# alexrenz/AdaPM

Measured on AMD Instinct MI355X. Metric: pull_push_ops_per_s, higher is better.
Workload: dtype fp32; 1 GPU; model=kge_complex_dim512, entities=10000000, relations=1000, dim=512, neg_samples=16, global_batch=16384, triples=90000000, parallelism=ps-async-dp1, fused_step=True, warmup_extra_steps=400

## Files before the change

### adapm_amd/csrc/core.cpp

```cpp
#include <torch/extension.h>
#include <ATen/Parallel.h>

#include <algorithm>
#include <atomic>
#include <condition_variable>
#include <cstring>
#include <limits>
#include <deque>
#include <map>
#include <queue>
#include <tuple>
#include <memory>
#include <mutex>
#include <random>
#include <thread>
#include <chrono>
#include <unordered_map>
#include <unordered_set>
#include <cstdio>
#include <vector>

#include "common.h"
#include "kernels.h"
#include "ops.h"
// ... 2385 lines not shown
  std::string failed_reason() {
    std::lock_guard<std::mutex> g(tickets_mu_);
    return failed_reason_;
  }

  void sync_finish(int ch, bool globally_idle = false) {
    if (globally_idle) {
      std::lock_guard<std::mutex> g(channels_[ch].mu);
      if (!channels_[ch].responses.empty()) globally_idle = false;
      for (const auto& r : channels_[ch].out_queue) {
        bool data = (r.payload.defined() && r.payload.numel() > 0) ||
                    r.code == M_PUSH_REQ || r.code == M_SET_REQ || r.code == M_PUSH_REQ_BULK;
        if (data) {
          globally_idle = false;
          break;
        }
      }
    }
    {
      std::lock_guard<std::mutex> g(rounds_mu_);
      ChannelState& C = channels_[ch];
      C.rounds++;
      if (globally_idle) {
        if (++C.idle_streak >= 2) C.idle2_events++;
      } else {
        C.idle_streak = 0;
      }
    }
    rounds_cv_.notify_all();
  }

  py::dict debug_pending() {
    py::dict d;
    {
      std::lock_guard<std::mutex> g(tickets_mu_);
      d["tickets"] = tickets_.size();
    }
    py::list outq, respq, rounds;
    for (auto& C : channels_) {
      std::lock_guard<std::mutex> g(C.mu);
      outq.append(C.out_queue.size());
      respq.append(C.responses.size());
      rounds.append(C.rounds.load());
    }
    d["out_queues"] = outq;
    d["responses"] = respq;
    d["rounds"] = rounds;
    return d;
  }


  bool fused_plain_ok(void* st) {
    if (clocks_.size() != 1 || fused_multi_stream_) return false;
    if (!fused_marks_.defined()) {
      if (getenv("ADAPM_FUSED_ATOMIC")) {
        fused_multi_stream_ = true;
        return false;
      }
      fused_marks_ = torch::zeros({rowmark_words(num_keys_)},
                                  torch::TensorOptions().dtype(torch::kInt32).device(dev_));
      if (getenv("ADAPM_FUSED_STATS"))
        fused_shared_stat_ =
            torch::zeros({1}, torch::TensorOptions().dtype(torch::kInt64).device(dev_));
      fused_marks_stream_ = st;
      return true;
    }
    if (st == fused_marks_stream_) return true;
#ifdef ADAPM_WITH_HIP
    hipStreamSynchronize((hipStream_t)fused_marks_stream_);
#endif
    fused_multi_stream_ = true;
    return false;
  }

  void check_fused_identity(const char* name, int64_t D) {
    TORCH_CHECK(world_ == 1, name, " requires a single rank (all keys local)");
    TORCH_CHECK(uniform_len_ == 2 * D, name, ": store rows must be [emb|accum] = 2D");
    TORCH_CHECK(layout_identity_.load(), name, " requires the identity layout");
    TORCH_CHECK(dev_.is_cuda(), name, " is the GPU fast path");
  }

  void count_fused_ops(int64_t keys) {
    stat_pull_keys_ += keys;
    stat_pull_local_ += keys;
    stat_push_keys_ += keys;
    stat_push_local_ += keys;
    stat_pulls_ += 1;
    stat_pushes_ += 1;
  }

  struct StagedKeys {
    torch::Tensor dev;
    std::vector<const int64_t*> ptr;
  };
  StagedKeys stage_keys(const char* name, std::initializer_list<const torch::Tensor*> parts) {
    int64_t total = 0;
    for (auto* t : parts) {
      check_keys(*t);
      total += t->numel();
    }
    auto blob = torch::empty(
        {total}, torch::TensorOptions().dtype(torch::kInt64).pinned_memory(true));
    int64_t* dst = blob.data_ptr<int64_t>();
    const uint64_t lim = (uint64_t)num_keys_;
    uint64_t bad = 0;
    for (auto* t : parts) {
      const int64_t* kp = t->data_ptr<int64_t>();
      const int64_t n = t->numel();
      for (int64_t i = 0; i < n; ++i) {
        int64_t k = kp[i];
        dst[i] = k;
        bad |= ((uint64_t)k >= lim);
      }
      dst += n;
    }
    if (bad)
      for (auto* t : parts) check_key_range(*t);
    StagedKeys sk;
    sk.dev = torch::empty({total}, torch::TensorOptions().dtype(torch::kInt64).device(dev_));
#ifdef ADAPM_WITH_HIP
    auto stream = c10::hip::getCurrentHIPStreamMasqueradingAsCUDA(dev_.index());
    TORCH_CHECK(copy_keys_gpu(sk.dev.data_ptr<int64_t>(), blob.data_ptr<int64_t>(), total,
                              (void*)stream.stream()),
                name, ": the pinned key staging buffer is not visible to the device");
    at::getHostAllocator(at::kCUDA)->record_event(
        blob.data_ptr(), blob.storage().data_ptr().get_context(), stream.unwrap());
#else
    TORCH_CHECK(false, name, ": built without HIP");
#endif
    const int64_t* dp = sk.dev.data_ptr<int64_t>();
    for (auto* t : parts) {
      sk.ptr.push_back(dp);
      dp += t->numel();
    }
    return sk;
  }

  std::tuple<torch::Tensor, torch::Tensor> kge_step_fused_impl(
      const torch::Tensor& keys_s, const torch::Tensor& keys_r, const torch::Tensor& keys_o,
      const torch::Tensor* keys_neg, UniformStream* us, int64_t N, int64_t D, double lr,
      double eps) {
    check_fused_identity("kge_step_fused", D);
    check_step_lanes("kge_step_fused", "D/2", D / 2);
    int64_t B = keys_s.numel();
    TORCH_CHECK(keys_r.numel() == B && keys_o.numel() == B);
    StagedKeys sk;
    torch::Tensor drawn;
    const int64_t* kn;
    if (us) {
      TORCH_CHECK(us->lo() >= 0 && us->hi() <= num_keys_, "kge_step_fused_sampled: stream range [",
                  us->lo(), ", ", us->hi(), ") exceeds the store's ", num_keys_, " keys");
      TORCH_CHECK(us->device() == dev_,
                  "kge_step_fused_sampled: stream is not on the store's device");
      TORCH_CHECK(N >= 0 && B * N > 0, "kge_step_fused_sampled: nothing to draw");
      sk = stage_keys("kge_step_fused", {&keys_s, &keys_r, &keys_o});
      drawn = us->draw(B * N);
      kn = drawn.data_ptr<int64_t>();
    } else {
      TORCH_CHECK(keys_neg->numel() == B * N);
      sk = stage_keys("kge_step_fused", {&keys_s, &keys_r, &keys_o, keys_neg});
      kn = sk.ptr[3];
    }
    const int64_t *ks = sk.ptr[0], *kr = sk.ptr[1], *ko = sk.ptr[2];

    auto loss = torch::empty({B}, torch::TensorOptions().dtype(torch::kFloat32).device(dev_));
    void* st = current_stream(dev_);
    {
      InflightGuard g(this);
      std::unique_lock<std::mutex> mg(fused_mu_);
      if (fused_plain_ok(st)) {
        RowMarkKeys mk{{ks, kr, ko, kn}, {B, B, B, B * N}, 4};
        auto* marks = reinterpret_cast<uint32_t*>(fused_marks_.data_ptr<int32_t>());
        rowmark_set_gpu(marks, mk, st);
        kge_complex_step_fused_gpu(
            slab_.data, mk.keys[0], mk.keys[1], mk.keys[2], mk.keys[3], loss.data_ptr<float>(),
            (int)B, (int)N, (int)D, Slab::padded(uniform_len_), world_, (float)lr, (float)eps,
            st, marks,
            fused_shared_stat_.defined()
                ? reinterpret_cast<unsigned long long*>(fused_shared_stat_.data_ptr<int64_t>())
                : nullptr);
        rowmark_clear_gpu(marks, mk, st);
        stat_fused_plain_ += 1;
      } else {
        mg.unlock();
        kge_complex_step_fused_gpu(slab_.data, ks, kr, ko, kn, loss.data_ptr<float>(), (int)B,
                                   (int)N, (int)D, Slab::padded(uniform_len_), world_, (float)lr,
                                   (float)eps, st);
        stat_fused_atomic_ += 1;
      }
    }
    count_fused_ops(3 * B + B * N);
    return {loss, drawn};
  }

  torch::Tensor kge_step_fused(torch::Tensor keys_s, torch::Tensor keys_r, torch::Tensor keys_o,
                               torch::Tensor keys_neg, int64_t N, int64_t D, double lr,
                               double eps) {
    return std::get<0>(
        kge_step_fused_impl(keys_s, keys_r, keys_o, &keys_neg, nullptr, N, D, lr, eps));
  }

  std::tuple<torch::Tensor, torch::Tensor> kge_step_fused_sampled(
      torch::Tensor keys_s, torch::Tensor keys_r, torch::Tensor keys_o, UniformStream& us,
      int64_t N, int64_t D, double lr, double eps) {
    return kge_step_fused_impl(keys_s, keys_r, keys_o, nullptr, &us, N, D, lr, eps);
  }

  struct FusedResolve {
    std::vector<std::vector<int64_t>> offs;
    std::vector<int64_t> missed;
    int64_t b_hit = 0;
    std::vector<const int64_t*> ptr;
    std::vector<torch::Tensor> dev;
  };

  FusedResolve resolve_fused(const std::vector<std::pair<const int64_t*, int>>& arrs,
                             int64_t B) {
    FusedResolve out;
    const int na = (int)arrs.size();
    constexpr int64_t G = 1024;
    int64_t nchunks = (B + G - 1) / G;
    struct Part {
      std::vector<std::vector<int64_t>> offs;
      std::vector<int64_t> missed;
    };
    std::vector<Part> parts(nchunks);
    pass_pool_.run(nchunks, [&](int64_t c0, int64_t c1) {
      for (int64_t c = c0; c < c1; ++c) {
        Part& P = parts[c];
        P.offs.resize(na);
        int64_t e = std::min(B, (c + 1) * G);
        std::vector<int64_t> tmp;
        for (int64_t b = c * G; b < e; ++b) {
          tmp.clear();
          bool ok = true;
          for (int a = 0; a < na && ok; ++a) {
            const int64_t* kp = arrs[a].first;
            int cnt = arrs[a].second;
            for (int i = 0; i < cnt; ++i) {
              Key k = kp[b * cnt + i];
// ... 563 lines not shown
  std::vector<ChannelState> channels_;
  std::unique_ptr<std::atomic<uint16_t>[]> intent_cnt_;
  std::vector<std::atomic<Clock>> clocks_;
  Clock intent_ahead_ = 1LL << 40;

  std::atomic<bool> layout_identity_{true};

  std::atomic<int> inflight_{0};
  int max_hops_ = getenv("ADAPM_MAX_HOPS") ? atoi(getenv("ADAPM_MAX_HOPS")) : 64;
  PassPool pass_pool_;
  std::atomic<int> migrating_{0};
  double sync_threshold_ = 0.0;
  std::unique_ptr<std::atomic<uint32_t>[]> heat_;
  std::mutex spill_mu_;
  std::mutex rebalance_mu_;
  std::vector<Key> spill_touched_;
  int64_t rebalance_calls_ = 0;
  std::atomic<int64_t> stat_spill_moves_{0};
  std::atomic<int64_t> next_ts_{1};
 public:
  std::atomic<int64_t> t_pass_{0}, t_todev_{0}, t_launch_{0}, t_calls_{0}, t_misc_{0};
  std::atomic<int64_t> t_sy_intents_{0}, t_sy_replicas_{0}, t_sy_build_{0}, t_sy_proc_{0},
      t_sy_apply_{0}, n_sy_deltas_{0}, n_sy_proc_recs_{0}, n_sy_apply_recs_{0};
  bool cpp_timing_ = getenv("ADAPM_CPP_TIMING") != nullptr;
 private:
  std::mutex tickets_mu_;
  std::condition_variable tickets_cv_;
  std::unordered_map<int64_t, std::unique_ptr<Ticket>> tickets_;
  std::unordered_map<int64_t, std::string> failed_tickets_;
  std::string failed_reason_;
  std::atomic<bool> failed_flag_{false};
  std::mutex rounds_mu_;
  std::condition_variable rounds_cv_;

  bool locality_stats_ = false;
  std::vector<std::atomic<uint32_t>> key_accesses_, key_local_;
  std::mutex trace_mu_;
  std::unordered_set<Key> traced_keys_;
  bool trace_all_ = false;
  struct TraceEv { double t; Key k; const char* ev; };
  std::vector<TraceEv> trace_;
  std::chrono::steady_clock::time_point t0_ = std::chrono::steady_clock::now();

  std::atomic<int64_t> hop_hist_[9] = {};
  std::atomic<int64_t> stat_replica_records_{0}, stat_replica_payloads_{0};
  std::atomic<int64_t> stat_pulls_{0}, stat_pushes_{0}, stat_pull_keys_{0}, stat_push_keys_{0},
      stat_pull_local_{0}, stat_push_local_{0}, stat_pull_replica_{0}, stat_push_replica_{0},
      stat_remote_pulls_served_{0}, stat_remote_pushes_served_{0}, stat_relocations_{0},
      stat_relocated_in_{0}, stat_replications_{0}, stat_drops_{0}, stat_forwards_{0},
      stat_dropped_records_{0}, stat_delta_overhops_{0}, stat_bytes_sent_{0},
      stat_bytes_recv_{0}, stat_sampling_checks_{0};

  std::mutex fused_mu_;
  torch::Tensor fused_marks_;
  torch::Tensor fused_shared_stat_;
  void* fused_marks_stream_ = nullptr;
  bool fused_multi_stream_ = false;
  std::atomic<int64_t> stat_fused_plain_{0}, stat_fused_atomic_{0};
};


static float* fp(torch::Tensor& t) { return t.data_ptr<float>(); }
static const float* cfp(const torch::Tensor& t) { return t.data_ptr<float>(); }

static void check_f32(const torch::Tensor& t, const char* name) {
  TORCH_CHECK(t.is_contiguous() && t.scalar_type() == torch::kFloat32, name,
              " must be contiguous float32");
}

void kge_complex_step(torch::Tensor s, torch::Tensor r, torch::Tensor o, torch::Tensor neg,
                      torch::Tensor ds, torch::Tensor dr, torch::Tensor do_, torch::Tensor dneg,
                      torch::Tensor loss, int64_t N, int64_t D, double lr, double eps) {
  for (auto* t : {&s, &r, &o, &neg, &ds, &dr, &do_, &dneg, &loss}) check_f32(*t, "kge tensor");
  int B = (int)loss.numel();
  if (s.is_cuda()) {
    TORCH_CHECK(hip_available(), "kge_complex_step: CUDA tensor but no HIP device");
    check_step_lanes("kge_complex_step", "D/2", D / 2);
    kge_complex_step_gpu(cfp(s), cfp(r), cfp(o), cfp(neg), fp(ds), fp(dr), fp(do_), fp(dneg),
                         fp(loss), B, (int)N, (int)D, (float)lr, (float)eps,
                         current_stream(s.device()));
  } else {
    kge_complex_step_cpu(cfp(s), cfp(r), cfp(o), cfp(neg), fp(ds), fp(dr), fp(do_), fp(dneg),
                         fp(loss), B, (int)N, (int)D, (float)lr, (float)eps);
  }
}

void rescal_step(torch::Tensor s, torch::Tensor r, torch::Tensor o, torch::Tensor neg,
                 torch::Tensor ds, torch::Tensor drl, torch::Tensor do_, torch::Tensor dneg,
                 torch::Tensor loss, int64_t N, int64_t D, double lr, double eps) {
  for (auto* t : {&s, &r, &o, &neg, &ds, &drl, &do_, &dneg, &loss}) check_f32(*t, "rescal");
  int B = (int)loss.numel();
  TORCH_CHECK(D <= 196, "rescal_step: dim must be <= 196 (R tile staged in LDS)");
  if (s.is_cuda()) {
    TORCH_CHECK(hip_available(), "rescal_step: CUDA tensor but no HIP device");
    rescal_step_gpu(cfp(s), cfp(r), cfp(o), cfp(neg), fp(ds), fp(drl), fp(do_), fp(dneg),
                    fp(loss), B, (int)N, (int)D, (float)lr, (float)eps,
                    current_stream(s.device()));
  } else {
    rescal_step_cpu(cfp(s), cfp(r), cfp(o), cfp(neg), fp(ds), fp(drl), fp(do_), fp(dneg),
                    fp(loss), B, (int)N, (int)D, (float)lr, (float)eps);
  }
}

void kge_complex_score(torch::Tensor s, torch::Tensor r, torch::Tensor cand,
                       torch::Tensor scores, int64_t D) {
  for (auto* t : {&s, &r, &cand, &scores}) check_f32(*t, "kge tensor");
  int B = (int)scores.size(0), E = (int)scores.size(1);
  if (s.is_cuda()) {
    TORCH_CHECK(hip_available(), "kge_complex_score: CUDA tensor but no HIP device");
// ... 214 lines not shown
  auto up = [&](const torch::Tensor& t) { return gpu ? t.to(dev.device()) : t; };
  torch::Tensor s_d = up(src_off), d_d = up(dst_off), l_d = up(lens), a_d;
  if (has_aux) a_d = up(*aux_off);
  OpsBatch b{s_d.data_ptr<int64_t>(), d_d.data_ptr<int64_t>(), l_d.data_ptr<int32_t>(), (int)n};
  const int64_t* a = has_aux ? a_d.data_ptr<int64_t>() : nullptr;
  float* bp = has_buf ? buf->data_ptr<float>() : nullptr;
  void* st = current_stream(dev.device());
  switch (kind) {
    case GATHER: gpu ? ops_gather_gpu(sb, b, bp, st) : ops_gather_cpu(sb, b, bp); break;
    case SCATTER: gpu ? ops_scatter_gpu(sb, b, bp, set, st) : ops_scatter_cpu(sb, b, bp, set); break;
    case RMW: ops_scatter_rmw_gpu(sb, b, bp, st); break;
    case EXTRACT: gpu ? ops_extract_gpu(sb, b, a, bp, st) : ops_extract_cpu(sb, b, a, bp); break;
    case REFRESH: gpu ? ops_refresh_gpu(sb, b, a, bp, st) : ops_refresh_cpu(sb, b, a, bp); break;
    case ZERO: gpu ? ops_zero_gpu(sb, b, st) : ops_zero_cpu(sb, b); break;
    case SQNORM: gpu ? ops_delta_sqnorm_gpu(sb, b, a, bp, st) : ops_delta_sqnorm_cpu(sb, b, a, bp); break;
  }
}

void slab_keys_op(const std::string& op, torch::Tensor dev, torch::Tensor keys, int64_t len,
                  int64_t plen, int64_t world, int64_t rank, torch::Tensor buf, bool set) {
  const bool gather = op == "gather_keys";
  TORCH_CHECK(gather || op == "scatter_keys", "slab_keys_op: unknown op '", op, "'");
  TORCH_CHECK(!(gather && set), "slab_keys_op: set applies to scatter_keys only");
  const bool gpu = dev.is_cuda();
  TORCH_CHECK(!gpu || hip_available(), "slab_keys_op: CUDA tensor but no HIP device");
  check_slab_tensor(dev, torch::kFloat32, "dev slab");
  check_slab_tensor(buf, torch::kFloat32, "buf");
  TORCH_CHECK(buf.device() == dev.device(), "slab_keys_op: buf and dev on different devices");
  const int64_t n = keys.numel();
  check_host_batch_tensor(keys, torch::kInt64, n, "keys");
  TORCH_CHECK(n <= std::numeric_limits<int>::max(), "slab_keys_op: batch too large");
  TORCH_CHECK(len >= 1 && plen >= len && plen <= std::numeric_limits<int32_t>::max(),
              "slab_keys_op: need 1 <= len <= plen");
  TORCH_CHECK((len & 3) != 0 || (plen & 3) == 0, "slab_keys_op: len % 4 == 0 needs plen % 4 == 0");
  TORCH_CHECK(world >= 1 && rank >= 0 && rank < world, "slab_keys_op: bad world / rank");
  TORCH_CHECK(n * len <= buf.numel(), "slab_keys_op: buf holds fewer than n rows");
  const int64_t* kp = keys.data_ptr<int64_t>();
  const int64_t rows = dev.numel() / plen;
  for (int64_t i = 0; i < n; ++i) {
    TORCH_CHECK(kp[i] >= 0, "slab_keys_op: keys[", i, "] is negative");
    TORCH_CHECK(kp[i] % world != rank || kp[i] / world < rows, "slab_keys_op: keys[", i, "] = ",
                kp[i], " lies past the slab's ", rows, " slots");
  }
  torch::Tensor k_d = gpu ? keys.to(dev.device()) : keys;
  SlabBases sb{dev.data_ptr<float>(), nullptr};
  KeyBatch b{k_d.data_ptr<int64_t>(), (int)n, (int32_t)len, (int32_t)plen, (int)world, (int)rank};
  void* st = current_stream(dev.device());
  if (gather)
    gpu ? ops_gather_keys_gpu(sb, b, fp(buf), st) : ops_gather_keys_cpu(sb, b, fp(buf));
  else
    gpu ? ops_scatter_keys_gpu(sb, b, cfp(buf), set, st) : ops_scatter_keys_cpu(sb, b, cfp(buf), set);
}

}

PYBIND11_MODULE(TORCH_EXTENSION_NAME, m) {
  using namespace adapm;
  m.def("hip_available", &hip_available);
  m.def("kge_complex_step", &kge_complex_step, py::call_guard<py::gil_scoped_release>());
  m.def("alias_draw", &alias_draw, py::call_guard<py::gil_scoped_release>());
  m.def("rescal_step", &rescal_step, py::call_guard<py::gil_scoped_release>());
  m.def("rescal_step_grouped", &rescal_step_grouped, py::call_guard<py::gil_scoped_release>());
  m.def("kge_complex_score", &kge_complex_score, py::call_guard<py::gil_scoped_release>());
  m.def("w2v_sgns_step", &w2v_sgns_step, py::call_guard<py::gil_scoped_release>());
  m.def("mf_update_step", &mf_update_step, py::call_guard<py::gil_scoped_release>());
  m.def("mf_loss", &mf_loss, py::call_guard<py::gil_scoped_release>());
  m.def("slab_op", &slab_op, py::arg("op"), py::arg("dev"), py::arg("host"), py::arg("src_off"),
        py::arg("dst_off"), py::arg("lens"), py::arg("aux_off"), py::arg("buf"), py::arg("set"),
        py::call_guard<py::gil_scoped_release>());
  m.def("slab_keys_op", &slab_keys_op, py::arg("op"), py::arg("dev"), py::arg("keys"),
        py::arg("len"), py::arg("plen"), py::arg("world"), py::arg("rank"), py::arg("buf"),
        py::arg("set"), py::call_guard<py::gil_scoped_release>());
  py::class_<UniformStream>(m, "UniformStream")
      .def(py::init<int64_t, int64_t, std::string>(), py::arg("lo"), py::arg("hi"),
           py::arg("device"))
      .def_static("supported", &UniformStream::supported)
      .def("import_state", &UniformStream::import_state, py::call_guard<py::gil_scoped_release>())
      .def("export_state", &UniformStream::export_state, py::call_guard<py::gil_scoped_release>())
      .def("draw", &UniformStream::draw, py::arg("n"), py::arg("slack") = -1,
           py::call_guard<py::gil_scoped_release>())
      .def("lo", &UniformStream::lo)
      .def("hi", &UniformStream::hi);
  py::class_<Server>(m, "Server")
      .def(py::init<int64_t, torch::Tensor, int, int, int, int, std::string, double, int, bool,
                    int64_t, int64_t, double>(),
           py::arg("num_keys"), py::arg("value_lengths"), py::arg("rank"), py::arg("world"),
           py::arg("num_channels"), py::arg("num_workers"), py::arg("device"),
           py::arg("capacity_factor") = 2.0, py::arg("techniques") = 0,
           py::arg("location_caches") = true, py::arg("device_cap_floats") = 0,
           py::arg("host_spill_floats") = 0, py::arg("sync_threshold") = 0.0)
      .def("pull", &Server::pull, py::call_guard<py::gil_scoped_release>())
      .def("push", &Server::push, py::call_guard<py::gil_scoped_release>())
      .def("pull_if_local", &Server::pull_if_local, py::call_guard<py::gil_scoped_release>())
      .def("is_local", &Server::is_local)
      .def("intent", &Server::intent, py::call_guard<py::gil_scoped_release>())
      .def("advance_clock", &Server::advance_clock)
      .def("current_clock", &Server::current_clock)
      .def("worker_clocks", &Server::worker_clocks)
      .def("wait", &Server::wait, py::call_guard<py::gil_scoped_release>())
      .def("wait_all", &Server::wait_all, py::call_guard<py::gil_scoped_release>())
      .def("is_finished", &Server::is_finished)
      .def("round_counts", &Server::round_counts)
      .def("wait_rounds", &Server::wait_rounds, py::call_guard<py::gil_scoped_release>())
      .def("idle_counts", &Server::idle_counts)
      .def("wait_idle", &Server::wait_idle, py::call_guard<py::gil_scoped_release>())
      .def("set_intent_ahead", &Server::set_intent_ahead)
      .def("sync_collect", &Server::sync_collect, py::call_guard<py::gil_scoped_release>())
      .def("sync_process", &Server::sync_process, py::call_guard<py::gil_scoped_release>())
      .def("sync_respond", &Server::sync_respond, py::call_guard<py::gil_scoped_release>())
      .def("sync_apply", &Server::sync_apply, py::call_guard<py::gil_scoped_release>())
      .def("sync_finish", &Server::sync_finish, py::arg("ch"),
           py::arg("globally_idle") = false, py::call_guard<py::gil_scoped_release>())
      .def("fail", &Server::fail, py::call_guard<py::gil_scoped_release>())
      .def("failed_reason", &Server::failed_reason)
      .def("scan_local", &Server::scan_local, py::call_guard<py::gil_scoped_release>())
      .def("kge_step_fused", &Server::kge_step_fused, py::call_guard<py::gil_scoped_release>())
      .def("kge_step_fused_sampled", &Server::kge_step_fused_sampled,
           py::call_guard<py::gil_scoped_release>())
      .def("w2v_step_fused", &Server::w2v_step_fused, py::call_guard<py::gil_scoped_release>())
      .def("mf_step_fused", &Server::mf_step_fused, py::call_guard<py::gil_scoped_release>())
      .def("kge_step_fused_general", &Server::kge_step_fused_general,
           py::call_guard<py::gil_scoped_release>())
      .def("w2v_step_fused_general", &Server::w2v_step_fused_general,
           py::call_guard<py::gil_scoped_release>())
      .def("mf_step_fused_general", &Server::mf_step_fused_general,
// ... 23 lines not shown
```

### adapm_amd/csrc/kernels.h

```cpp
#pragma once
#include <cstdint>

namespace adapm {

constexpr int STEP_MAX_LANES = 8 * 256;

void kge_complex_step_gpu(const float* s, const float* r, const float* o, const float* neg,
                          float* ds, float* dr, float* do_, float* dneg, float* loss,
                          int B, int N, int D, float lr, float eps, void* stream);
void kge_complex_step_cpu(const float* s, const float* r, const float* o, const float* neg,
                          float* ds, float* dr, float* do_, float* dneg, float* loss,
                          int B, int N, int D, float lr, float eps);

struct RowMarkKeys {
  const int64_t* keys[4];
  int64_t n[4];
  int count;
};
inline int64_t rowmark_words(int64_t rows) { return (rows + 15) / 16; }
void rowmark_set_gpu(uint32_t* marks, const RowMarkKeys& ks, void* stream);
void rowmark_clear_gpu(uint32_t* marks, const RowMarkKeys& ks, void* stream);

void kge_complex_step_fused_gpu(float* slab, const int64_t* keys_s, const int64_t* keys_r,
                                const int64_t* keys_o, const int64_t* keys_neg, float* loss,
                                int B, int N, int D, int32_t plen, int world, float lr,
                                float eps, void* stream, const uint32_t* marks = nullptr,
                                unsigned long long* shared_stat = nullptr);

void kge_complex_step_fused_offs_cpu(float* slab, const int64_t* offs_s, const int64_t* offs_r,
                                     const int64_t* offs_o, const int64_t* offs_neg, float* loss,
                                     int B, int N, int D, float lr, float eps);
void w2v_sgns_step_fused_offs_cpu(float* slab, const int64_t* offs_ctr, const int64_t* offs_ctx,
                                  const int64_t* offs_neg, float* loss, int B, int N, int D,
                                  float lr, float eps);
void mf_update_step_fused_offs_cpu(float* slab, const int64_t* offs_w, const int64_t* offs_h,
                                   const float* x, float* loss, int B, int R, float lr,
                                   float lambda, float eps);

void w2v_sgns_step_fused_gpu(float* slab, const int64_t* keys_ctr, const int64_t* keys_ctx,
                             const int64_t* keys_neg, float* loss, int B, int N, int D,
                             int32_t plen, int world, float lr, float eps, void* stream);

void mf_update_step_fused_gpu(float* slab, const int64_t* keys_w, const int64_t* keys_h,
                              const float* x, float* loss, int B, int R, int32_t plen,
                              int world, float lr, float lambda, float eps, void* stream);

void kge_complex_score_gpu(const float* s, const float* r, const float* cand, float* scores,
                           int B, int E, int D, void* stream);
void kge_complex_score_cpu(const float* s, const float* r, const float* cand, float* scores,
                           int B, int E, int D);

void rescal_step_gpu(const float* s, const float* r, const float* o, const float* neg,
                     float* ds, float* drl, float* do_, float* dneg, float* loss, int B, int N,
                     int D, float lr, float eps, void* stream);
void rescal_step_cpu(const float* s, const float* r, const float* o, const float* neg,
                     float* ds, float* drl, float* do_, float* dneg, float* loss, int B, int N,
                     int D, float lr, float eps);

void w2v_sgns_step_gpu(const float* ctr, const float* ctx, const float* neg, float* dctr,
                       float* dctx, float* dneg, float* loss, int B, int N, int D, float lr,
                       float eps, void* stream);
void w2v_sgns_step_cpu(const float* ctr, const float* ctx, const float* neg, float* dctr,
                       float* dctx, float* dneg, float* loss, int B, int N, int D, float lr,
                       float eps);

void mf_update_step_gpu(const float* w, const float* h, const float* x, float* dw, float* dh,
                        float* loss, int B, int R, float lr, float lambda, float eps,
                        void* stream);
void mf_update_step_cpu(const float* w, const float* h, const float* x, float* dw, float* dh,
                        float* loss, int B, int R, float lr, float lambda, float eps);

void mf_loss_gpu(const float* w, const float* h, const float* x, double* acc2, int B, int R,
                 float lambda, void* stream);
void mf_loss_cpu(const float* w, const float* h, const float* x, float* out2, int B, int R,
                 float lambda);

void alias_draw_gpu(const float* prob, const int32_t* alias, int64_t n, uint64_t seed,
                    int64_t N, int64_t* out, void* stream);
void alias_draw_cpu(const float* prob, const int32_t* alias, int64_t n, uint64_t seed,
// ... 31 lines not shown
```

### adapm_amd/csrc/kernels_hip.hip

```cpp
#include <hip/hip_runtime.h>
#include <algorithm>
#include <type_traits>

#include "kernels.h"
#include "ustream.h"

namespace adapm {

#define KT 256

static inline unsigned grid_for(int64_t n, int64_t cap = 16384) {
  return (unsigned)std::min(std::max<int64_t>(n, 1), cap);
}

static_assert(STEP_MAX_LANES == 8 * KT, "dispatch_kpt stops at KPT = 8");
template <typename F>
static inline void dispatch_kpt(int lanes, F&& f) {
  if (lanes <= KT) f(std::integral_constant<int, 1>{});
  else if (lanes <= 2 * KT) f(std::integral_constant<int, 2>{});
  else if (lanes <= 4 * KT) f(std::integral_constant<int, 4>{});
  else f(std::integral_constant<int, 8>{});
}

__device__ inline float block_reduce_sum(float v, float* lds) {
// ... 460 lines not shown
    float lsum = 0.f;
    for (int j = 0; j <= N; ++j) {
      const float* ob = (j == 0) ? o + (int64_t)b * erow
                                 : neg + ((int64_t)b * N + j - 1) * erow;
      float* dob = (j == 0) ? do_ + (int64_t)b * erow
                            : dneg + ((int64_t)b * N + j - 1) * erow;
      float y = (j == 0) ? 1.f : -1.f;
      float part = 0.f;
      for (int k = threadIdx.x; k < D; k += KT) part += u[k] * ob[k];
      float dot = block_reduce_sum(part, red);
      float c = -y * sigmoidf(-y * dot);
      if (threadIdx.x == 0) lsum += softplusf(-y * dot);
      for (int k = threadIdx.x; k < D; k += KT) {
        w[k] += c * ob[k];
        write_delta(&dob[k], &dob[D + k], c * u[k], ob[D + k], lr, eps);
      }
      __syncthreads();
    }
    if (threadIdx.x == 0) loss[b] = lsum;

    float* dsb = ds + (int64_t)b * erow;
    for (int i = threadIdx.x; i < D; i += KT) {
      float a = 0.f;
      for (int k = 0; k < D; ++k) a += Rm[i * D + k] * w[k];
      write_delta(&dsb[i], &dsb[D + i], a, sb[D + i], lr, eps);
    }
    float* drb = drl + (int64_t)b * rrow;
    for (int idx = threadIdx.x; idx < D * D; idx += KT) {
      int i = idx / D, k = idx % D;
      const int64_t acc = (int64_t)D * D + idx;
      write_delta(&drb[idx], &drb[acc], es[i] * w[k], rb[acc], lr, eps);
    }
    __syncthreads();
  }
}

void rescal_step_gpu(const float* s, const float* r, const float* o, const float* neg,
                     float* ds, float* drl, float* do_, float* dneg, float* loss, int B, int N,
                     int D, float lr, float eps, void* stream) {
  size_t smem = (size_t)(D * D + 3 * D + KT / 64) * sizeof(float);
  if (B < 1) return;
  hipLaunchKernelGGL(k_rescal_step, dim3(grid_for(B, 8192)), dim3(KT), smem, (hipStream_t)stream,
                     s, r, o, neg, ds, drl, do_, dneg, loss, B, N, D, lr, eps);
}

}

namespace adapm {

__device__ inline float* row_at(float* slab, int64_t v, int32_t plen, int world) {
  return world ? slab + (v / world) * (int64_t)plen : slab + v;
}

__device__ inline uint32_t* rowmark_word(uint32_t* marks, int64_t row) { return marks + (row >> 4); }
__device__ inline int rowmark_shift(int64_t row) { return 2 * (int)(row & 15); }

__device__ inline int64_t rowmark_key(const RowMarkKeys& ks, int64_t i) {
  int a = 0;
  while (a < ks.count - 1 && i >= ks.n[a]) {
    i -= ks.n[a];
    ++a;
  }
  return ks.keys[a][i];
}

__global__ void k_rowmark_set(uint32_t* __restrict__ marks, RowMarkKeys ks, int64_t total) {
  int64_t i = (int64_t)blockIdx.x * blockDim.x + threadIdx.x;
  if (i >= total) return;
  int64_t row = rowmark_key(ks, i);
  uint32_t bit = 1u << rowmark_shift(row);
  uint32_t old = atomicOr(rowmark_word(marks, row), bit);
  if ((old & bit) && !(old & (bit << 1))) atomicOr(rowmark_word(marks, row), bit << 1);
}

__global__ void k_rowmark_clear(uint32_t* __restrict__ marks, RowMarkKeys ks, int64_t total) {
  int64_t i = (int64_t)blockIdx.x * blockDim.x + threadIdx.x;
  if (i >= total) return;
  *rowmark_word(marks, rowmark_key(ks, i)) = 0u;
}

void rowmark_set_gpu(uint32_t* marks, const RowMarkKeys& ks, void* stream) {
  int64_t total = 0;
  for (int a = 0; a < ks.count; ++a) total += ks.n[a];
  if (total == 0) return;
  hipLaunchKernelGGL(k_rowmark_set, dim3((unsigned)((total + KT - 1) / KT)), dim3(KT), 0,
                     (hipStream_t)stream, marks, ks, total);
}

void rowmark_clear_gpu(uint32_t* marks, const RowMarkKeys& ks, void* stream) {
  int64_t total = 0;
  for (int a = 0; a < ks.count; ++a) total += ks.n[a];
  if (total == 0) return;
  hipLaunchKernelGGL(k_rowmark_clear, dim3((unsigned)((total + KT - 1) / KT)), dim3(KT), 0,
                     (hipStream_t)stream, marks, ks, total);
}

template <bool UNIQ>
__device__ inline bool row_shared(const uint32_t* __restrict__ marks, int64_t key) {
  if (!UNIQ) return true;
  return (marks[key >> 4] >> (rowmark_shift(key) + 1)) & 1u;
}

__device__ inline float plain_add(float a, float delta) {
#pragma clang fp contract(off)
  return a + delta;
}

__device__ inline void slab_adagrad(float* p_emb, float* p_acc, float g, float emb, float acc,
                                    float lr, float eps, bool shared) {
  float d = adagrad_delta(g, acc, lr, eps);
  if (shared) {
    atomicAdd(p_emb, d);
    atomicAdd(p_acc, g * g);
  } else {
    *p_emb = plain_add(emb, d);
    *p_acc = plain_add(acc, g * g);
  }
}

#define SLAB_ADAGRAD_COMPLEX(row, shared, g_re, g_im, emb_re, emb_im, acc_re, acc_im) \
  do {                                                                                \
    float G_re = (acc_re) + (g_re) * (g_re);                                          \
    float G_im = (acc_im) + (g_im) * (g_im);                                          \
    float d_re = -lr * (g_re) * __frsqrt_rn(G_re + eps);                              \
    float d_im = -lr * (g_im) * __frsqrt_rn(G_im + eps);                              \
    if (shared) {                                                                     \
      atomicAdd(&(row)[k], d_re);                                                     \
      atomicAdd(&(row)[dc + k], d_im);                                                \
      atomicAdd(&(row)[D + k], (g_re) * (g_re));                                      \
      atomicAdd(&(row)[D + dc + k], (g_im) * (g_im));                                 \
    } else {                                                                          \
      (row)[k] = plain_add(emb_re, d_re);                                             \
      (row)[dc + k] = plain_add(emb_im, d_im);                                        \
      (row)[D + k] = plain_add(acc_re, (g_re) * (g_re));                              \
      (row)[D + dc + k] = plain_add(acc_im, (g_im) * (g_im));                         \
    }                                                                                 \
  } while (0)

template <int KPT, bool UNIQ>
__global__ void k_kge_step_fused(float* __restrict__ slab, const int64_t* __restrict__ keys_s,
                                 const int64_t* __restrict__ keys_r,
                                 const int64_t* __restrict__ keys_o,
                                 const int64_t* __restrict__ keys_neg, float* __restrict__ loss,
                                 int B, int N, int D, int32_t plen, int world, float lr,
                                 float eps, const uint32_t* __restrict__ marks,
                                 unsigned long long* __restrict__ shared_stat) {
  __shared__ float lds[KT / 64];
  const int dc = D >> 1;
  const int w = UNIQ ? 1 : world;
  for (int b = blockIdx.x; b < B; b += gridDim.x) {
    const int64_t key_s = keys_s[b], key_r = keys_r[b];
    const float* sb = row_at(slab, key_s, plen, w);
    const float* rb = row_at(slab, key_r, plen, w);
    const bool s_shared = row_shared<UNIQ>(marks, key_s);
    const bool r_shared = row_shared<UNIQ>(marks, key_r);
    unsigned n_shared = (unsigned)s_shared + (unsigned)r_shared;

    float s_re[KPT], s_im[KPT], r_re[KPT], r_im[KPT];
    float a_sre[KPT], a_sim[KPT], a_rre[KPT], a_rim[KPT];
    float u_re[KPT], u_im[KPT];
#pragma unroll
    for (int i = 0; i < KPT; ++i) {
      int k = threadIdx.x + i * KT;
      a_sre[i] = a_sim[i] = a_rre[i] = a_rim[i] = 0.f;
      if (k < dc) {
        s_re[i] = sb[k];
        s_im[i] = sb[dc + k];
        r_re[i] = rb[k];
        r_im[i] = rb[dc + k];
        u_re[i] = s_re[i] * r_re[i] - s_im[i] * r_im[i];
        u_im[i] = s_im[i] * r_re[i] + s_re[i] * r_im[i];
      } else {
        s_re[i] = s_im[i] = r_re[i] = r_im[i] = u_re[i] = u_im[i] = 0.f;
      }
    }

    float lsum = 0.f;
    for (int j = 0; j <= N; ++j) {
      int64_t ok = (j == 0) ? keys_o[b] : keys_neg[(int64_t)b * N + (j - 1)];
      float* ob = row_at(slab, ok, plen, w);
      const bool o_shared = row_shared<UNIQ>(marks, ok);
      n_shared += (unsigned)o_shared;
      float y = (j == 0) ? 1.f : -1.f;
      float part = 0.f;
      float o_re[KPT], o_im[KPT], Go_re[KPT], Go_im[KPT];
#pragma unroll
      for (int i = 0; i < KPT; ++i) {
        int k = threadIdx.x + i * KT;
        o_re[i] = k < dc ? ob[k] : 0.f;
        o_im[i] = k < dc ? ob[dc + k] : 0.f;
        Go_re[i] = k < dc ? ob[D + k] : 0.f;
        Go_im[i] = k < dc ? ob[D + dc + k] : 0.f;
        part += u_re[i] * o_re[i] + u_im[i] * o_im[i];
      }
      float psi = block_reduce_sum(part, lds);
      float c = -y * sigmoidf(-y * psi);
      if (threadIdx.x == 0) lsum += softplusf(-y * psi);

#pragma unroll
      for (int i = 0; i < KPT; ++i) {
        int k = threadIdx.x + i * KT;
        if (k >= dc) continue;
        a_sre[i] += c * (r_re[i] * o_re[i] + r_im[i] * o_im[i]);
        a_sim[i] += c * (r_re[i] * o_im[i] - r_im[i] * o_re[i]);
        a_rre[i] += c * (s_re[i] * o_re[i] + s_im[i] * o_im[i]);
        a_rim[i] += c * (s_re[i] * o_im[i] - s_im[i] * o_re[i]);
        float g_re = c * u_re[i];
        float g_im = c * u_im[i];
        SLAB_ADAGRAD_COMPLEX(ob, o_shared, g_re, g_im, o_re[i], o_im[i], Go_re[i], Go_im[i]);
      }
    }
    float* dsb = const_cast<float*>(sb);
    float* drb = const_cast<float*>(rb);
#pragma unroll
    for (int i = 0; i < KPT; ++i) {
      int k = threadIdx.x + i * KT;
      if (k >= dc) continue;
      float Gs_re = sb[D + k], Gs_im = sb[D + dc + k];
      SLAB_ADAGRAD_COMPLEX(dsb, s_shared, a_sre[i], a_sim[i], s_re[i], s_im[i], Gs_re, Gs_im);
      float Gr_re = rb[D + k], Gr_im = rb[D + dc + k];
      SLAB_ADAGRAD_COMPLEX(drb, r_shared, a_rre[i], a_rim[i], r_re[i], r_im[i], Gr_re, Gr_im);
    }
    if (threadIdx.x == 0) {
      loss[b] = lsum;
      if (UNIQ && shared_stat) atomicAdd(shared_stat, (unsigned long long)n_shared);
    }
  }
}

#undef SLAB_ADAGRAD_COMPLEX

void kge_complex_step_fused_gpu(float* slab, const int64_t* keys_s, const int64_t* keys_r,
                                const int64_t* keys_o, const int64_t* keys_neg, float* loss,
                                int B, int N, int D, int32_t plen, int world, float lr,
                                float eps, void* stream, const uint32_t* marks,
                                unsigned long long* shared_stat) {
  if (B < 1) return;
  const bool uniq = marks != nullptr && world == 1;
  if (!uniq) marks = nullptr, shared_stat = nullptr;
  dispatch_kpt(D >> 1, [&](auto kpt) {
    constexpr int KPT = decltype(kpt)::value;
    hipLaunchKernelGGL((uniq ? k_kge_step_fused<KPT, true> : k_kge_step_fused<KPT, false>),
                       dim3(grid_for(B)), dim3(KT), 0, (hipStream_t)stream, slab, keys_s, keys_r,
                       keys_o, keys_neg, loss, B, N, D, plen, world, lr, eps, marks,
                       shared_stat);
  });
}

}

namespace adapm {

template <int KPT>
__global__ void k_w2v_step_fused(float* __restrict__ slab, const int64_t* __restrict__ keys_ctr,
                                 const int64_t* __restrict__ keys_ctx,
                                 const int64_t* __restrict__ keys_neg, float* __restrict__ loss,
                                 int B, int N, int D, int32_t plen, int world, float lr,
                                 float eps) {
  __shared__ float lds[KT / 64];
  for (int b = blockIdx.x; b < B; b += gridDim.x) {
    float* cb = row_at(slab, keys_ctr[b], plen, world);
    float c_emb[KPT], a_c[KPT];
#pragma unroll
    for (int i = 0; i < KPT; ++i) {
      int k = threadIdx.x + i * KT;
      c_emb[i] = k < D ? cb[k] : 0.f;
      a_c[i] = 0.f;
    }
    float lsum = 0.f;
    for (int j = 0; j <= N; ++j) {
      int64_t xk = (j == 0) ? keys_ctx[b] : keys_neg[(int64_t)b * N + (j - 1)];
      float* xb = row_at(slab, xk, plen, world);
      float y = (j == 0) ? 1.f : -1.f;
      float part = 0.f;
      float x_emb[KPT];
#pragma unroll
      for (int i = 0; i < KPT; ++i) {
        int k = threadIdx.x + i * KT;
        x_emb[i] = k < D ? xb[k] : 0.f;
        part += c_emb[i] * x_emb[i];
      }
      float dot = block_reduce_sum(part, lds);
      float g = -y * sigmoidf(-y * dot);
      if (threadIdx.x == 0) lsum += softplusf(-y * dot);
#pragma unroll
      for (int i = 0; i < KPT; ++i) {
        int k = threadIdx.x + i * KT;
        if (k >= D) continue;
        a_c[i] += g * x_emb[i];
        slab_adagrad(&xb[k], &xb[D + k], g * c_emb[i], x_emb[i], xb[D + k], lr, eps,
                     true);
      }
    }
#pragma unroll
    for (int i = 0; i < KPT; ++i) {
      int k = threadIdx.x + i * KT;
      if (k >= D) continue;
// ... 49 lines not shown
```

Before: 1.220 billion key-ops/s.

## Replace atomic row marks with occurrence-index tags fused into key upload

The per-step duplicate-row detection no longer uses atomicOr on 2-bit marks followed by a clear pass. Each occurrence now writes its index into a per-row tag array, fused into the kernel that copies keys from pinned memory. A flag pass then marks any row whose tag disagrees as shared, and a bits pass compacts this into a 1-bit-per-row mask the step kernel reads. This drops the clear kernel and the atomics, and folds the key copy into the tagging kernel. The cost is a tag array of 32 words per 32 rows and an extra bits kernel, and the logic relies on last-writer-wins tag semantics being correct across a launch boundary.

New measurement: 1.282 billion key-ops/s (median of 6 runs). 5.1% higher.

```diff
diff --git a/adapm_amd/csrc/core.cpp b/adapm_amd/csrc/core.cpp
--- a/adapm_amd/csrc/core.cpp
+++ b/adapm_amd/csrc/core.cpp
@@ -2461,22 +2461,22 @@
 
   bool fused_plain_ok(void* st) {
     if (clocks_.size() != 1 || fused_multi_stream_) return false;
-    if (!fused_marks_.defined()) {
+    if (!fused_tags_.defined()) {
       if (getenv("ADAPM_FUSED_ATOMIC")) {
         fused_multi_stream_ = true;
         return false;
       }
-      fused_marks_ = torch::zeros({rowmark_words(num_keys_)},
-                                  torch::TensorOptions().dtype(torch::kInt32).device(dev_));
+      fused_tags_ = torch::empty({33 * rowtag_words(num_keys_)},
+                                 torch::TensorOptions().dtype(torch::kInt32).device(dev_));
       if (getenv("ADAPM_FUSED_STATS"))
         fused_shared_stat_ =
             torch::zeros({1}, torch::TensorOptions().dtype(torch::kInt64).device(dev_));
-      fused_marks_stream_ = st;
+      fused_tags_stream_ = st;
       return true;
     }
-    if (st == fused_marks_stream_) return true;
+    if (st == fused_tags_stream_) return true;
 #ifdef ADAPM_WITH_HIP
-    hipStreamSynchronize((hipStream_t)fused_marks_stream_);
+    hipStreamSynchronize((hipStream_t)fused_tags_stream_);
 #endif
     fused_multi_stream_ = true;
     return false;
@@ -2498,14 +2498,24 @@
     stat_pushes_ += 1;
   }
 
+  struct HostKeys {
+    torch::Tensor blob;
+    std::vector<int64_t> n;
+  };
   struct StagedKeys {
     torch::Tensor dev;
     std::vector<const int64_t*> ptr;
   };
   StagedKeys stage_keys(const char* name, std::initializer_list<const torch::Tensor*> parts) {
+    return upload_keys(name, host_keys(parts));
+  }
+
+  HostKeys host_keys(std::initializer_list<const torch::Tensor*> parts) {
+    HostKeys hk;
     int64_t total = 0;
     for (auto* t : parts) {
       check_keys(*t);
+      hk.n.push_back(t->numel());
       total += t->numel();
     }
     auto blob = torch::empty(
@@ -2525,22 +2535,33 @@
     }
     if (bad)
       for (auto* t : parts) check_key_range(*t);
+    hk.blob = blob;
+    return hk;
+  }
+
+  StagedKeys upload_keys(const char* name, const HostKeys& hk, uint32_t* tags = nullptr,
+                         const int64_t* dev_keys = nullptr, int64_t n_dev = 0) {
+    const torch::Tensor& blob = hk.blob;
+    const int64_t total = blob.numel();
     StagedKeys sk;
     sk.dev = torch::empty({total}, torch::TensorOptions().dtype(torch::kInt64).device(dev_));
 #ifdef ADAPM_WITH_HIP
     auto stream = c10::hip::getCurrentHIPStreamMasqueradingAsCUDA(dev_.index());
-    TORCH_CHECK(copy_keys_gpu(sk.dev.data_ptr<int64_t>(), blob.data_ptr<int64_t>(), total,
-                              (void*)stream.stream()),
-                name, ": the pinned key staging buffer is not visible to the device");
+    const bool ok =
+        tags ? keys_land_gpu(tags, sk.dev.data_ptr<int64_t>(), blob.data_ptr<int64_t>(), total,
+                             dev_keys, n_dev, (void*)stream.stream())
+             : copy_keys_gpu(sk.dev.data_ptr<int64_t>(), blob.data_ptr<int64_t>(), total,
+                             (void*)stream.stream());
+    TORCH_CHECK(ok, name, ": the pinned key staging buffer is not visible to the device");
     at::getHostAllocator(at::kCUDA)->record_event(
         blob.data_ptr(), blob.storage().data_ptr().get_context(), stream.unwrap());
 #else
     TORCH_CHECK(false, name, ": built without HIP");
 #endif
     const int64_t* dp = sk.dev.data_ptr<int64_t>();
-    for (auto* t : parts) {
+    for (int64_t n : hk.n) {
       sk.ptr.push_back(dp);
-      dp += t->numel();
+      dp += n;
     }
     return sk;
   }
@@ -2553,24 +2574,26 @@
     check_step_lanes("kge_step_fused", "D/2", D / 2);
     int64_t B = keys_s.numel();
     TORCH_CHECK(keys_r.numel() == B && keys_o.numel() == B);
+    TORCH_CHECK(N >= 0 && (3 + N) * B < (int64_t)ROWTAG_SHARED,
+                "kge_step_fused: too many keys in one step");
+    HostKeys hk;
     StagedKeys sk;
     torch::Tensor drawn;
-    const int64_t* kn;
+    const int64_t* kn = nullptr;
     if (us) {
       TORCH_CHECK(us->lo() >= 0 && us->hi() <= num_keys_, "kge_step_fused_sampled: stream range [",
                   us->lo(), ", ", us->hi(), ") exceeds the store's ", num_keys_, " keys");
       TORCH_CHECK(us->device() == dev_,
                   "kge_step_fused_sampled: stream is not on the store's device");
       TORCH_CHECK(N >= 0 && B * N > 0, "kge_step_fused_sampled: nothing to draw");
-      sk = stage_keys("kge_step_fused", {&keys_s, &keys_r, &keys_o});
+      hk = host_keys({&keys_s, &keys_r, &keys_o});
       drawn = us->draw(B * N);
       kn = drawn.data_ptr<int64_t>();
     } else {
       TORCH_CHECK(keys_neg->numel() == B * N);
-      sk = stage_keys("kge_step_fused", {&keys_s, &keys_r, &keys_o, keys_neg});
-      kn = sk.ptr[3];
-    }
-    const int64_t *ks = sk.ptr[0], *kr = sk.ptr[1], *ko = sk.ptr[2];
+      hk = host_keys({&keys_s, &keys_r, &keys_o, keys_neg});
+    }
+    const int64_t n_dev = us ? B * N : 0;
 
     auto loss = torch::empty({B}, torch::TensorOptions().dtype(torch::kFloat32).device(dev_));
     void* st = current_stream(dev_);
@@ -2578,23 +2601,27 @@
       InflightGuard g(this);
       std::unique_lock<std::mutex> mg(fused_mu_);
       if (fused_plain_ok(st)) {
-        RowMarkKeys mk{{ks, kr, ko, kn}, {B, B, B, B * N}, 4};
-        auto* marks = reinterpret_cast<uint32_t*>(fused_marks_.data_ptr<int32_t>());
-        rowmark_set_gpu(marks, mk, st);
+        auto* tags = reinterpret_cast<uint32_t*>(fused_tags_.data_ptr<int32_t>());
+        uint32_t* bits = tags + 32 * rowtag_words(num_keys_);
+        sk = upload_keys("kge_step_fused", hk, tags, kn, n_dev);
+        if (!us) kn = sk.ptr[3];
+        RowTagKeys tk{{sk.ptr[0], kn, nullptr, nullptr}, {hk.blob.numel(), n_dev, 0, 0}, 2};
+        rowtag_flag_gpu(tags, tk, st);
+        rowtag_bits_gpu(tags, bits, tk, st);
         kge_complex_step_fused_gpu(
-            slab_.data, mk.keys[0], mk.keys[1], mk.keys[2], mk.keys[3], loss.data_ptr<float>(),
-            (int)B, (int)N, (int)D, Slab::padded(uniform_len_), world_, (float)lr, (float)eps,
-            st, marks,
+            slab_.data, sk.ptr[0], sk.ptr[1], sk.ptr[2], kn, loss.data_ptr<float>(), (int)B,
+            (int)N, (int)D, Slab::padded(uniform_len_), world_, (float)lr, (float)eps, st, bits,
             fused_shared_stat_.defined()
                 ? reinterpret_cast<unsigned long long*>(fused_shared_stat_.data_ptr<int64_t>())
                 : nullptr);
-        rowmark_clear_gpu(marks, mk, st);
         stat_fused_plain_ += 1;
       } else {
         mg.unlock();
-        kge_complex_step_fused_gpu(slab_.data, ks, kr, ko, kn, loss.data_ptr<float>(), (int)B,
-                                   (int)N, (int)D, Slab::padded(uniform_len_), world_, (float)lr,
-                                   (float)eps, st);
+        sk = upload_keys("kge_step_fused", hk);
+        if (!us) kn = sk.ptr[3];
+        kge_complex_step_fused_gpu(slab_.data, sk.ptr[0], sk.ptr[1], sk.ptr[2], kn,
+                                   loss.data_ptr<float>(), (int)B, (int)N, (int)D,
+                                   Slab::padded(uniform_len_), world_, (float)lr, (float)eps, st);
         stat_fused_atomic_ += 1;
       }
     }
@@ -3264,9 +3291,9 @@
       stat_bytes_recv_{0}, stat_sampling_checks_{0};
 
   std::mutex fused_mu_;
-  torch::Tensor fused_marks_;
+  torch::Tensor fused_tags_;
   torch::Tensor fused_shared_stat_;
-  void* fused_marks_stream_ = nullptr;
+  void* fused_tags_stream_ = nullptr;
   bool fused_multi_stream_ = false;
   std::atomic<int64_t> stat_fused_plain_{0}, stat_fused_atomic_{0};
 };
@@ -3587,6 +3614,39 @@
     gpu ? ops_scatter_keys_gpu(sb, b, cfp(buf), set, st) : ops_scatter_keys_cpu(sb, b, cfp(buf), set);
 }
 
+torch::Tensor rowtag_shared_mask(std::vector<torch::Tensor> keys, int64_t num_keys) {
+  TORCH_CHECK(hip_available(), "rowtag_shared_mask: no HIP device");
+  TORCH_CHECK(!keys.empty() && keys.size() <= 4, "rowtag_shared_mask: one to four key arrays");
+  TORCH_CHECK(num_keys >= 1 && num_keys <= std::numeric_limits<int32_t>::max(),
+              "rowtag_shared_mask: bad num_keys");
+  const torch::Device dev(torch::kCUDA, c10::hip::current_device());
+  std::vector<torch::Tensor> dk;
+  RowTagKeys tk{{nullptr, nullptr, nullptr, nullptr}, {0, 0, 0, 0}, (int)keys.size()};
+  int64_t total = 0;
+  for (size_t a = 0; a < keys.size(); ++a) {
+    const int64_t n = keys[a].numel();
+    check_host_batch_tensor(keys[a], torch::kInt64, n, "keys");
+    const int64_t* kp = keys[a].data_ptr<int64_t>();
+    for (int64_t i = 0; i < n; ++i)
+      TORCH_CHECK(kp[i] >= 0 && kp[i] < num_keys, "rowtag_shared_mask: key out of range: ", kp[i]);
+    dk.push_back(keys[a].to(dev));
+    tk.keys[a] = dk.back().data_ptr<int64_t>();
+    tk.n[a] = n;
+    total += n;
+  }
+  TORCH_CHECK(total < (int64_t)ROWTAG_SHARED, "rowtag_shared_mask: too many occurrences");
+  const int64_t words = rowtag_words(num_keys);
+  auto tags = torch::empty({33 * words}, torch::TensorOptions().dtype(torch::kInt32).device(dev));
+  auto* tp = reinterpret_cast<uint32_t*>(tags.data_ptr<int32_t>());
+  void* st = current_stream(dev);
+  rowtag_tag_gpu(tp, tk, st);
+  rowtag_flag_gpu(tp, tk, st);
+  rowtag_bits_gpu(tp, tp + 32 * words, tk, st);
+  auto all = torch::cat(dk);
+  auto word = tags.narrow(0, 32 * words, words).index_select(0, all.div(32, "floor"));
+  return word.bitwise_right_shift(all.remainder(32).to(torch::kInt32)).bitwise_and(1).eq(1);
+}
+
 }
 
 PYBIND11_MODULE(TORCH_EXTENSION_NAME, m) {
@@ -3606,6 +3666,8 @@
   m.def("slab_keys_op", &slab_keys_op, py::arg("op"), py::arg("dev"), py::arg("keys"),
         py::arg("len"), py::arg("plen"), py::arg("world"), py::arg("rank"), py::arg("buf"),
         py::arg("set"), py::call_guard<py::gil_scoped_release>());
+  m.def("rowtag_shared_mask", &rowtag_shared_mask, py::arg("keys"), py::arg("num_keys"),
+        py::call_guard<py::gil_scoped_release>());
   py::class_<UniformStream>(m, "UniformStream")
       .def(py::init<int64_t, int64_t, std::string>(), py::arg("lo"), py::arg("hi"),
            py::arg("device"))
diff --git a/adapm_amd/csrc/kernels.h b/adapm_amd/csrc/kernels.h
--- a/adapm_amd/csrc/kernels.h
+++ b/adapm_amd/csrc/kernels.h
@@ -12,19 +12,24 @@
                           float* ds, float* dr, float* do_, float* dneg, float* loss,
                           int B, int N, int D, float lr, float eps);
 
-struct RowMarkKeys {
+constexpr uint32_t ROWTAG_SHARED = 0xFFFFFFFFu;
+struct RowTagKeys {
   const int64_t* keys[4];
   int64_t n[4];
   int count;
 };
-inline int64_t rowmark_words(int64_t rows) { return (rows + 15) / 16; }
-void rowmark_set_gpu(uint32_t* marks, const RowMarkKeys& ks, void* stream);
-void rowmark_clear_gpu(uint32_t* marks, const RowMarkKeys& ks, void* stream);
+inline int64_t rowtag_words(int64_t rows) { return (rows + 31) / 32; }
+void rowtag_tag_gpu(uint32_t* tags, const RowTagKeys& ks, void* stream);
+void rowtag_flag_gpu(uint32_t* tags, const RowTagKeys& ks, void* stream);
+void rowtag_bits_gpu(const uint32_t* tags, uint32_t* bits, const RowTagKeys& ks, void* stream);
+
+bool keys_land_gpu(uint32_t* tags, int64_t* dst, const int64_t* src_host, int64_t n_copy,
+                   const int64_t* dev_keys, int64_t n_dev, void* stream);
 
 void kge_complex_step_fused_gpu(float* slab, const int64_t* keys_s, const int64_t* keys_r,
                                 const int64_t* keys_o, const int64_t* keys_neg, float* loss,
                                 int B, int N, int D, int32_t plen, int world, float lr,
-                                float eps, void* stream, const uint32_t* marks = nullptr,
+                                float eps, void* stream, const uint32_t* bits = nullptr,
                                 unsigned long long* shared_stat = nullptr);
 
 void kge_complex_step_fused_offs_cpu(float* slab, const int64_t* offs_s, const int64_t* offs_r,
diff --git a/adapm_amd/csrc/kernels_hip.hip b/adapm_amd/csrc/kernels_hip.hip
--- a/adapm_amd/csrc/kernels_hip.hip
+++ b/adapm_amd/csrc/kernels_hip.hip
@@ -536,10 +536,7 @@
   return world ? slab + (v / world) * (int64_t)plen : slab + v;
 }
 
-__device__ inline uint32_t* rowmark_word(uint32_t* marks, int64_t row) { return marks + (row >> 4); }
-__device__ inline int rowmark_shift(int64_t row) { return 2 * (int)(row & 15); }
-
-__device__ inline int64_t rowmark_key(const RowMarkKeys& ks, int64_t i) {
+__device__ inline int64_t rowtag_key(const RowTagKeys& ks, int64_t i) {
   int a = 0;
   while (a < ks.count - 1 && i >= ks.n[a]) {
     i -= ks.n[a];
@@ -548,41 +545,105 @@
   return ks.keys[a][i];
 }
 
-__global__ void k_rowmark_set(uint32_t* __restrict__ marks, RowMarkKeys ks, int64_t total) {
-  int64_t i = (int64_t)blockIdx.x * blockDim.x + threadIdx.x;
+__device__ inline void rowtag_tag(uint32_t* tags, int64_t row, int64_t i) {
+  tags[row] = (uint32_t)i;
+}
+
+__device__ inline void rowtag_flag(uint32_t* tags, int64_t row, int64_t i) {
+  if (tags[row] != (uint32_t)i) tags[row] = ROWTAG_SHARED;
+}
+
+__global__ void k_keys_land(uint32_t* __restrict__ tags, int64_t* __restrict__ dst,
+                            const int64_t* __restrict__ src, int64_t n_copy,
+                            const int64_t* __restrict__ dev_keys, int64_t total) {
+  int64_t i = (int64_t)blockIdx.x * KT + threadIdx.x;
   if (i >= total) return;
-  int64_t row = rowmark_key(ks, i);
-  uint32_t bit = 1u << rowmark_shift(row);
-  uint32_t old = atomicOr(rowmark_word(marks, row), bit);
-  if ((old & bit) && !(old & (bit << 1))) atomicOr(rowmark_word(marks, row), bit << 1);
-}
-
-__global__ void k_rowmark_clear(uint32_t* __restrict__ marks, RowMarkKeys ks, int64_t total) {
-  int64_t i = (int64_t)blockIdx.x * blockDim.x + threadIdx.x;
+  int64_t row;
+  if (i < n_copy) {
+    row = src[i];
+    dst[i] = row;
+  } else {
+    row = dev_keys[i - n_copy];
+  }
+  rowtag_tag(tags, row, i);
+}
+
+__global__ void k_rowtag_tag(uint32_t* __restrict__ tags, RowTagKeys ks, int64_t total) {
+  int64_t i = (int64_t)blockIdx.x * KT + threadIdx.x;
   if (i >= total) return;
-  *rowmark_word(marks, rowmark_key(ks, i)) = 0u;
-}
-
-void rowmark_set_gpu(uint32_t* marks, const RowMarkKeys& ks, void* stream) {
+  rowtag_tag(tags, rowtag_key(ks, i), i);
+}
+
+__global__ void k_rowtag_flag(uint32_t* __restrict__ tags, RowTagKeys ks, int64_t total) {
+  int64_t i = (int64_t)blockIdx.x * KT + threadIdx.x;
+  if (i >= total) return;
+  rowtag_flag(tags, rowtag_key(ks, i), i);
+}
+
+__global__ void k_rowtag_bits(const uint32_t* __restrict__ tags, uint32_t* __restrict__ bits,
+                              RowTagKeys ks, int64_t total) {
+  int64_t i = (int64_t)blockIdx.x * KT + threadIdx.x;
+  if (i >= total) return;
+  const int64_t w = rowtag_key(ks, i) >> 5;
+  const uint4* t = reinterpret_cast<const uint4*>(tags + (w << 5));
+  uint32_t word = 0;
+#pragma unroll
+  for (int q = 0; q < 8; ++q) {
+    const uint4 v = t[q];
+    word |= ((uint32_t)(v.x == ROWTAG_SHARED) | (uint32_t)(v.y == ROWTAG_SHARED) << 1 |
+             (uint32_t)(v.z == ROWTAG_SHARED) << 2 | (uint32_t)(v.w == ROWTAG_SHARED) << 3)
+            << (4 * q);
+  }
+  bits[w] = word;
+}
+
+static int64_t rowtag_total(const RowTagKeys& ks) {
   int64_t total = 0;
   for (int a = 0; a < ks.count; ++a) total += ks.n[a];
+  return total;
+}
+
+void rowtag_tag_gpu(uint32_t* tags, const RowTagKeys& ks, void* stream) {
+  const int64_t total = rowtag_total(ks);
   if (total == 0) return;
-  hipLaunchKernelGGL(k_rowmark_set, dim3((unsigned)((total + KT - 1) / KT)), dim3(KT), 0,
-                     (hipStream_t)stream, marks, ks, total);
-}
-
-void rowmark_clear_gpu(uint32_t* marks, const RowMarkKeys& ks, void* stream) {
-  int64_t total = 0;
-  for (int a = 0; a < ks.count; ++a) total += ks.n[a];
+  hipLaunchKernelGGL(k_rowtag_tag, dim3((unsigned)((total + KT - 1) / KT)), dim3(KT), 0,
+                     (hipStream_t)stream, tags, ks, total);
+}
+
+void rowtag_flag_gpu(uint32_t* tags, const RowTagKeys& ks, void* stream) {
+  const int64_t total = rowtag_total(ks);
   if (total == 0) return;
-  hipLaunchKernelGGL(k_rowmark_clear, dim3((unsigned)((total + KT - 1) / KT)), dim3(KT), 0,
-                     (hipStream_t)stream, marks, ks, total);
+  hipLaunchKernelGGL(k_rowtag_flag, dim3((unsigned)((total + KT - 1) / KT)), dim3(KT), 0,
+                     (hipStream_t)stream, tags, ks, total);
+}
+
+void rowtag_bits_gpu(const uint32_t* tags, uint32_t* bits, const RowTagKeys& ks, void* stream) {
+  const int64_t total = rowtag_total(ks);
+  if (total == 0) return;
+  hipLaunchKernelGGL(k_rowtag_bits, dim3((unsigned)((total + KT - 1) / KT)), dim3(KT), 0,
+                     (hipStream_t)stream, tags, bits, ks, total);
+}
+
+bool keys_land_gpu(uint32_t* tags, int64_t* dst, const int64_t* src_host, int64_t n_copy,
+                   const int64_t* dev_keys, int64_t n_dev, void* stream) {
+  const int64_t total = n_copy + n_dev;
+  if (total <= 0) return true;
+  void* src = nullptr;
+  if (n_copy > 0 &&
+      (hipHostGetDevicePointer(&src, const_cast<int64_t*>(src_host), 0) != hipSuccess || !src)) {
+    (void)hipGetLastError();
+    return false;
+  }
+  hipLaunchKernelGGL(k_keys_land, dim3((unsigned)((total + KT - 1) / KT)), dim3(KT), 0,
+                     (hipStream_t)stream, tags, dst, static_cast<const int64_t*>(src), n_copy,
+                     dev_keys, total);
+  return true;
 }
 
 template <bool UNIQ>
-__device__ inline bool row_shared(const uint32_t* __restrict__ marks, int64_t key) {
+__device__ inline bool row_shared(const uint32_t* __restrict__ bits, int64_t key) {
   if (!UNIQ) return true;
-  return (marks[key >> 4] >> (rowmark_shift(key) + 1)) & 1u;
+  return (bits[key >> 5] >> (int)(key & 31)) & 1u;
 }
 
 __device__ inline float plain_add(float a, float delta) {
@@ -627,7 +688,7 @@
                                  const int64_t* __restrict__ keys_o,
                                  const int64_t* __restrict__ keys_neg, float* __restrict__ loss,
                                  int B, int N, int D, int32_t plen, int world, float lr,
-                                 float eps, const uint32_t* __restrict__ marks,
+                                 float eps, const uint32_t* __restrict__ bits,
                                  unsigned long long* __restrict__ shared_stat) {
   __shared__ float lds[KT / 64];
   const int dc = D >> 1;
@@ -636,8 +697,8 @@
     const int64_t key_s = keys_s[b], key_r = keys_r[b];
     const float* sb = row_at(slab, key_s, plen, w);
     const float* rb = row_at(slab, key_r, plen, w);
-    const bool s_shared = row_shared<UNIQ>(marks, key_s);
-    const bool r_shared = row_shared<UNIQ>(marks, key_r);
+    const bool s_shared = row_shared<UNIQ>(bits, key_s);
+    const bool r_shared = row_shared<UNIQ>(bits, key_r);
     unsigned n_shared = (unsigned)s_shared + (unsigned)r_shared;
 
     float s_re[KPT], s_im[KPT], r_re[KPT], r_im[KPT];
@@ -663,7 +724,7 @@
     for (int j = 0; j <= N; ++j) {
       int64_t ok = (j == 0) ? keys_o[b] : keys_neg[(int64_t)b * N + (j - 1)];
       float* ob = row_at(slab, ok, plen, w);
-      const bool o_shared = row_shared<UNIQ>(marks, ok);
+      const bool o_shared = row_shared<UNIQ>(bits, ok);
       n_shared += (unsigned)o_shared;
       float y = (j == 0) ? 1.f : -1.f;
       float part = 0.f;
@@ -717,16 +778,16 @@
 void kge_complex_step_fused_gpu(float* slab, const int64_t* keys_s, const int64_t* keys_r,
                                 const int64_t* keys_o, const int64_t* keys_neg, float* loss,
                                 int B, int N, int D, int32_t plen, int world, float lr,
-                                float eps, void* stream, const uint32_t* marks,
+                                float eps, void* stream, const uint32_t* bits,
                                 unsigned long long* shared_stat) {
   if (B < 1) return;
-  const bool uniq = marks != nullptr && world == 1;
-  if (!uniq) marks = nullptr, shared_stat = nullptr;
+  const bool uniq = bits != nullptr && world == 1;
+  if (!uniq) bits = nullptr, shared_stat = nullptr;
   dispatch_kpt(D >> 1, [&](auto kpt) {
     constexpr int KPT = decltype(kpt)::value;
     hipLaunchKernelGGL((uniq ? k_kge_step_fused<KPT, true> : k_kge_step_fused<KPT, false>),
                        dim3(grid_for(B)), dim3(KT), 0, (hipStream_t)stream, slab, keys_s, keys_r,
-                       keys_o, keys_neg, loss, B, N, D, plen, world, lr, eps, marks,
+                       keys_o, keys_neg, loss, B, N, D, plen, world, lr, eps, bits,
                        shared_stat);
   });
 }
```
